# facebookresearch/multipathnet

Measured on NVIDIA H100. Metric: proposals/sec, higher is better.
Workload: dtype fp32 (wgmma split emulation, fp32 accumulate: 3 bf16 products per MAC, 2 fp16 products in fc6/fc7)

## Files before the change

multipathnet_b200/csrc/gemm_tc.cu:

```cuda
#include "conv_gemm.cuh"
#include "wgmma.cuh"
#include <algorithm>
#include <stdlib.h>
#include <string.h>

namespace {

constexpr int BM = 128;
constexpr int BK = 64;
constexpr int TC_THREADS = 384;
constexpr int CONS_THREADS = 256;
constexpr int A_TILE_BYTES = BM * BK * 2;
constexpr int SMEM_BUDGET = 196608;

__host__ __device__ constexpr int stage_bytes(int BN, bool W16 = false) { return 2 * A_TILE_BYTES + (W16 ? 1 : 2) * BN * BK * 2; }
__host__ __device__ constexpr int num_stages(int BN, bool W16 = false) {
  return (SMEM_BUDGET / stage_bytes(BN, W16)) > 4 ? 4 : (SMEM_BUDGET / stage_bytes(BN, W16));
}
__host__ __device__ constexpr int stg_ld(int BN) { return BN + 4; }
static_assert(BM * (256 + 4) * 4 <= 2 * stage_bytes(256), "staging tile must fit in the ring");

struct TcParams {
  int N, Ho, Wo, Cout;
  int kh, kw, stride, pad;
  int cblocks;
  int tn, th, tw;
  int tiles_img, tiles_h, tiles_w, tiles_n;
  const float *bias;
  const __nv_bfloat16 *res_hi, *res_lo; long long res_ld;
  __nv_bfloat16 *out_hi, *out_lo; long long out_ld;
  float *out_f32; long long out_f32_ld;
  __nv_bfloat16 *pool_hi, *pool_lo; long long pool_ld; int Hp, Wp;
  int relu;
  int splitk, kb_per_split;
  long long split_stride;
  unsigned long long *tl_min, *tl_max;
  float acc_scale;
  int out_fmt;
  unsigned *ovf;
};

__device__ __forceinline__ unsigned long long gtimer() {
  unsigned long long t; asm volatile("mov.u64 %0, %%globaltimer;" : "=l"(t)); return t;
}
__device__ __forceinline__ void tl_min_stamp(const unsigned long long *base_, int i) {
  if (base_) atomicMin(const_cast<unsigned long long *>(base_) + i, gtimer());
}
__device__ __forceinline__ void tl_max_stamp(const unsigned long long *base_, int i) {
  if (base_) atomicMax(const_cast<unsigned long long *>(base_) + i, gtimer());
}
__device__ __forceinline__ uint32_t smem_u32(const void *p) { return (uint32_t)__cvta_generic_to_shared(p); }
__device__ __forceinline__ void mbar_init(uint32_t bar, uint32_t count) {
  asm volatile("mbarrier.init.shared::cta.b64 [%0], %1;" ::"r"(bar), "r"(count) : "memory");
}
__device__ __forceinline__ void mbar_expect_tx(uint32_t bar, uint32_t bytes) {
  asm volatile("mbarrier.arrive.expect_tx.shared::cta.b64 _, [%0], %1;" ::"r"(bar), "r"(bytes) : "memory");
}
__device__ __forceinline__ void mbar_arrive(uint32_t bar) {
  asm volatile("mbarrier.arrive.shared::cta.b64 _, [%0];" ::"r"(bar) : "memory");
}
__device__ __forceinline__ void mbar_wait(uint32_t bar, uint32_t parity) {
  uint32_t done;
  uint32_t spins = 0;
  do {
    asm volatile(
        "{\n\t.reg .pred p;\n\t"
        "mbarrier.try_wait.parity.shared::cta.b64 p, [%1], %2;\n\t"
        "selp.u32 %0, 1, 0, p;\n\t}"
        : "=r"(done) : "r"(bar), "r"(parity) : "memory");
    if (!done && ++spins == (1u << 26)) __trap();
  } while (!done);
}
__device__ __forceinline__ void tma_load_4d(uint32_t dst, const CUtensorMap *tm, uint32_t bar, int c0, int c1,
                                            int c2, int c3) {
  asm volatile(
      "cp.async.bulk.tensor.4d.shared::cluster.global.mbarrier::complete_tx::bytes [%0], [%1, {%3, %4, %5, %6}], [%2];"
      ::"r"(dst), "l"(reinterpret_cast<uint64_t>(tm)), "r"(bar), "r"(c0), "r"(c1), "r"(c2), "r"(c3) : "memory");
}
__device__ __forceinline__ void tma_load_2d(uint32_t dst, const CUtensorMap *tm, uint32_t bar, int c0, int c1) {
  asm volatile(
      "cp.async.bulk.tensor.2d.shared::cluster.global.mbarrier::complete_tx::bytes [%0], [%1, {%3, %4}], [%2];"
      ::"r"(dst), "l"(reinterpret_cast<uint64_t>(tm)), "r"(bar), "r"(c0), "r"(c1) : "memory");
}
__device__ __forceinline__ void prefetch_tmap(const CUtensorMap *tm) {
  asm volatile("prefetch.tensormap [%0];" ::"l"(reinterpret_cast<uint64_t>(tm)) : "memory");
}
__device__ __forceinline__ void consumers_sync() { asm volatile("bar.sync 1, 256;" ::: "memory"); }

__device__ __forceinline__ uint64_t make_smem_desc(uint32_t saddr) {
  uint64_t d = 0;
  d |= (uint64_t)((saddr & 0x3FFFFu) >> 4);
  d |= (uint64_t)1 << 16;
  d |= (uint64_t)(1024 >> 4) << 32;
  d |= (uint64_t)1 << 62;
  return d;
}

template <int BN, bool W16>
__device__ __forceinline__ void mma_kblock(float (&acc)[BN / 2], uint64_t a_hi, uint64_t a_lo, uint64_t b_hi, uint64_t b_lo, bool first) {
#pragma unroll
  for (int k = 0; k < BK / 16; ++k) {
    const uint64_t adv = (uint64_t)((k * 16 * 2) >> 4);
    const uint32_t later = (first && k == 0) ? 0u : 1u;
    wgmma_nk16<BN, W16>(acc, a_lo + adv, b_hi + adv, later);
    if (!W16) wgmma_nk16<BN, W16>(acc, a_hi + adv, b_lo + adv, 1u);
    wgmma_nk16<BN, W16>(acc, a_hi + adv, b_hi + adv, 1u);
  }
}

template <int BN>
__device__ __forceinline__ void stage_acc(float *stg, const float (&acc)[BN / 2], int g, int t) {
  const int r0 = g * 64 + (t >> 5) * 16 + ((t & 31) >> 2), c0 = 2 * (t & 3);
#pragma unroll
  for (int j = 0; j < BN / 8; ++j) {
    *reinterpret_cast<float2 *>(stg + r0 * stg_ld(BN) + 8 * j + c0) = make_float2(acc[4 * j], acc[4 * j + 1]);
    *reinterpret_cast<float2 *>(stg + (r0 + 8) * stg_ld(BN) + 8 * j + c0) = make_float2(acc[4 * j + 2], acc[4 * j + 3]);
  }
}

template <int BN, bool W16>
__device__ __forceinline__ void epilogue_row(const TcParams &p, const float *srow, int nt, bool row_ok, long long pix,
                                             float *out_f32, int ch_first, long long ppix) {
  const bool pool = (p.pool_hi != nullptr);
  const int tile_end = min(p.Cout, nt * BN + BN);
#pragma unroll 1
  for (int ch = ch_first; ch < BN / 32; ch += 2) {
    const int col0 = nt * BN + ch * 32;
    if (col0 >= tile_end) break;
    float v[32];
#pragma unroll
    for (int j = 0; j < 8; ++j) {
      const float4 x = *reinterpret_cast<const float4 *>(srow + ch * 32 + 4 * j);
      v[4 * j] = x.x; v[4 * j + 1] = x.y; v[4 * j + 2] = x.z; v[4 * j + 3] = x.w;
    }
    if (W16) {
#pragma unroll
      for (int e = 0; e < 32; ++e) v[e] *= p.acc_scale;
    }
    if (!(row_ok || pool)) continue;
#pragma unroll
    for (int g = 0; g < 4; ++g) {
      const int c = col0 + g * 8;
      if (c >= tile_end) break;
      float f[8];
#pragma unroll
      for (int e = 0; e < 8; ++e) f[e] = v[g * 8 + e];
      const bool full8 = (c + 8 <= tile_end);
      if (p.bias) {
        if (full8) {
          const float4 b0 = __ldg(reinterpret_cast<const float4 *>(p.bias + c));
          const float4 b1 = __ldg(reinterpret_cast<const float4 *>(p.bias + c + 4));
          f[0] += b0.x; f[1] += b0.y; f[2] += b0.z; f[3] += b0.w;
          f[4] += b1.x; f[5] += b1.y; f[6] += b1.z; f[7] += b1.w;
        } else {
          for (int e = 0; e < 8 && c + e < p.Cout; ++e) f[e] += __ldg(p.bias + c + e);
        }
      }
      if (p.res_hi && full8 && row_ok) {
        const uint4 rh = *reinterpret_cast<const uint4 *>(p.res_hi + pix * p.res_ld + c);
        const uint4 rl = *reinterpret_cast<const uint4 *>(p.res_lo + pix * p.res_ld + c);
        const uint32_t hh[4] = {rh.x, rh.y, rh.z, rh.w}, ll[4] = {rl.x, rl.y, rl.z, rl.w};
#pragma unroll
        for (int t = 0; t < 4; ++t) {
          float2 x = bf16x2_to_float2(hh[t]), y = bf16x2_to_float2(ll[t]);
          f[2 * t] += x.x + y.x; f[2 * t + 1] += x.y + y.y;
        }
      }
      if (p.relu) {
#pragma unroll
        for (int e = 0; e < 8; ++e) f[e] = fmaxf(f[e], 0.f);
      }
      if (p.out_hi && full8 && row_ok) {
        uint32_t oh[4], ol[4];
#pragma unroll
        for (int t = 0; t < 4; ++t) split_x2(p.out_fmt, f[2 * t], f[2 * t + 1], oh[t], ol[t], p.ovf);
        *reinterpret_cast<uint4 *>(p.out_hi + pix * p.out_ld + c) = make_uint4(oh[0], oh[1], oh[2], oh[3]);
        *reinterpret_cast<uint4 *>(p.out_lo + pix * p.out_ld + c) = make_uint4(ol[0], ol[1], ol[2], ol[3]);
      }
      if (pool) {
#pragma unroll
        for (int e = 0; e < 8; ++e) {
          float x = row_ok ? f[e] : -INFINITY;
          x = fmaxf(x, __shfl_xor_sync(0xffffffffu, x, 1));
          x = fmaxf(x, __shfl_xor_sync(0xffffffffu, x, 8));
          f[e] = x;
        }
        if (ppix >= 0 && full8) {
          uint32_t oh[4], ol[4];
#pragma unroll
          for (int t = 0; t < 4; ++t) split_x2(p.out_fmt, f[2 * t], f[2 * t + 1], oh[t], ol[t], p.ovf);
          *reinterpret_cast<uint4 *>(p.pool_hi + ppix * p.pool_ld + c) = make_uint4(oh[0], oh[1], oh[2], oh[3]);
          *reinterpret_cast<uint4 *>(p.pool_lo + ppix * p.pool_ld + c) = make_uint4(ol[0], ol[1], ol[2], ol[3]);
        }
      }
      if (out_f32 && row_ok) {
        float *o = out_f32 + pix * p.out_f32_ld + c;
        if (full8 && ((reinterpret_cast<uintptr_t>(o) & 15) == 0)) {
          reinterpret_cast<float4 *>(o)[0] = make_float4(f[0], f[1], f[2], f[3]);
          reinterpret_cast<float4 *>(o)[1] = make_float4(f[4], f[5], f[6], f[7]);
        } else {
          for (int e = 0; e < 8 && c + e < p.Cout; ++e) o[e] = f[e];
        }
      }
    }
  }
}

template <int BN, bool W16 = false>
__global__ void __launch_bounds__(TC_THREADS, 1)
conv_gemm_tc_kernel(const __grid_constant__ CUtensorMap tmA_hi, const __grid_constant__ CUtensorMap tmA_lo,
                    const __grid_constant__ CUtensorMap tmB_hi, const __grid_constant__ CUtensorMap tmB_lo,
                    const TcParams p) {
  constexpr int S = num_stages(BN, W16);
  constexpr int STAGE = stage_bytes(BN, W16);
  constexpr int B_TILE_BYTES = BN * BK * 2;
  static_assert(BM * stg_ld(BN) * 4 <= S * STAGE, "staging tile must fit in the ring");
  extern __shared__ uint8_t smem_raw[];
  uint8_t *smem = reinterpret_cast<uint8_t *>((reinterpret_cast<uintptr_t>(smem_raw) + 1023) & ~(uintptr_t)1023);
  uint64_t *bars = reinterpret_cast<uint64_t *>(smem + (size_t)S * STAGE);
  const uint32_t smem_base = smem_u32(smem);
  const uint32_t bar_base = smem_u32(bars);
  auto full_bar = [&](int s) { return bar_base + 8u * s; };
  auto empty_bar = [&](int s) { return bar_base + 8u * (S + s); };

  const int tid = threadIdx.x, lane = tid & 31;
  const int unit = (int)blockIdx.x;
  const int tile = unit / p.splitk, split = unit - tile * p.splitk;
  const int nt = tile % p.tiles_n, mt = tile / p.tiles_n;
  const int twi = mt % p.tiles_w, thi = (mt / p.tiles_w) % p.tiles_h, tni = mt / (p.tiles_w * p.tiles_h);
  const int num_kb = p.kh * p.kw * p.cblocks;
  const int kb0 = split * p.kb_per_split, kb1 = min(num_kb, kb0 + p.kb_per_split);

  if (tid == 0) {
    tl_min_stamp(p.tl_min, 0);
    prefetch_tmap(&tmA_hi); prefetch_tmap(&tmA_lo); prefetch_tmap(&tmB_hi); prefetch_tmap(&tmB_lo);
    for (int s = 0; s < S; ++s) { mbar_init(full_bar(s), 1); mbar_init(empty_bar(s), CONS_THREADS / 32); }
    asm volatile("fence.mbarrier_init.release.cluster;" ::: "memory");
  }
  __syncthreads();
  asm volatile("griddepcontrol.wait;" ::: "memory");
  asm volatile("griddepcontrol.launch_dependents;" ::: "memory");
  if (tid == 0) tl_min_stamp(p.tl_min, 1);

  if (tid < 128) {
    if (tid == 0) {
      const int w_in0 = twi * p.tw * p.stride - p.pad, h_in0 = thi * p.th * p.stride - p.pad, n0 = tni * p.tn;
      const int b_row0 = nt * BN;
      for (int kb = kb0, it = 0; kb < kb1; ++kb, ++it) {
        const int s = it % S; const uint32_t ph = (uint32_t)(it / S) & 1u;
        mbar_wait(empty_bar(s), ph ^ 1u);
        const int tap = kb / p.cblocks, cb = kb - tap * p.cblocks;
        const int khi = tap / p.kw, kwi = tap - khi * p.kw;
        const uint32_t sa = smem_base + (uint32_t)s * STAGE;
        mbar_expect_tx(full_bar(s), (uint32_t)STAGE);
        tma_load_4d(sa, &tmA_hi, full_bar(s), cb * BK, w_in0 + kwi, h_in0 + khi, n0);
        tma_load_4d(sa + A_TILE_BYTES, &tmA_lo, full_bar(s), cb * BK, w_in0 + kwi, h_in0 + khi, n0);
        tma_load_2d(sa + 2 * A_TILE_BYTES, &tmB_hi, full_bar(s), kb * BK, b_row0);
        if (!W16) tma_load_2d(sa + 2 * A_TILE_BYTES + B_TILE_BYTES, &tmB_lo, full_bar(s), kb * BK, b_row0);
      }
    }
    return;
  }

  const int e = tid - 128;
  const int g = e >> 7, t = e & 127;
  float acc[BN / 2];
#pragma unroll
  for (int i = 0; i < BN / 2; ++i) acc[i] = 0.f;
  for (int kb = kb0, it = 0; kb < kb1; ++kb, ++it) {
    const int s = it % S; const uint32_t ph = (uint32_t)(it / S) & 1u;
    mbar_wait(full_bar(s), ph);
    if (it == 0 && e == 0) tl_min_stamp(p.tl_min, 2);
    const uint32_t sa = smem_base + (uint32_t)s * STAGE;
    const uint64_t a_hi = make_smem_desc(sa + (uint32_t)g * (A_TILE_BYTES / 2));
    const uint64_t a_lo = make_smem_desc(sa + A_TILE_BYTES + (uint32_t)g * (A_TILE_BYTES / 2));
    const uint64_t b_hi = make_smem_desc(sa + 2 * A_TILE_BYTES);
    const uint64_t b_lo = make_smem_desc(sa + 2 * A_TILE_BYTES + B_TILE_BYTES);
    wgmma_fence_acc(acc);
    wgmma_fence();
    mma_kblock<BN, W16>(acc, a_hi, a_lo, b_hi, b_lo, it == 0);
    wgmma_commit();
    wgmma_wait<1>();
    wgmma_fence_acc(acc);
    if (it > 0 && lane == 0) mbar_arrive(empty_bar((it - 1) % S));
  }
  wgmma_wait<0>();
  wgmma_fence_acc(acc);
  if (e == 0) tl_max_stamp(p.tl_max, 0);
  consumers_sync();
  float *stg = reinterpret_cast<float *>(smem);
  stage_acc<BN>(stg, acc, g, t);
  consumers_sync();

  const int row = e & 127;
  const int wl = row & (p.tw - 1), hl = (row / p.tw) & (p.th - 1), nl = row / (p.tw * p.th);
  const int wo = twi * p.tw + wl, ho = thi * p.th + hl, n = tni * p.tn + nl;
  const bool row_ok = (wo < p.Wo) && (ho < p.Ho) && (n < p.N);
  const long long pix = ((long long)n * p.Ho + ho) * p.Wo + wo;
  const long long ppix = (p.pool_hi && row_ok && !(lane & 9)) ? ((long long)n * p.Hp + (ho >> 1)) * p.Wp + (wo >> 1) : -1;
  float *const out_f32 = p.out_f32 ? p.out_f32 + (long long)split * p.split_stride : nullptr;
  epilogue_row<BN, W16>(p, stg + row * stg_ld(BN), nt, row_ok, pix, out_f32, e >> 7, ppix);
  if (e == 0) tl_max_stamp(p.tl_max, 1);
}

constexpr int C1_THREADS = 256;
constexpr int C1_B_BYTES = 2 * 64 * 128;
constexpr int C1_SMEM = 2 * A_TILE_BYTES + C1_B_BYTES + BM * stg_ld(64) * 4 + 1024;

__global__ void __launch_bounds__(C1_THREADS, 2)
conv1_tc_kernel(const float *__restrict__ x, int N, int H, int W, const float *__restrict__ w, const TcParams p) {
  extern __shared__ uint8_t smem_raw[];
  uint8_t *smem = reinterpret_cast<uint8_t *>((reinterpret_cast<uintptr_t>(smem_raw) + 1023) & ~(uintptr_t)1023);
  uint8_t *sB = smem + 2 * A_TILE_BYTES;
  float *stg = reinterpret_cast<float *>(sB + C1_B_BYTES);
  const uint32_t a_base = smem_u32(smem), b_base = smem_u32(sB);
  const int tid = threadIdx.x, lane = tid & 31;
  const int g = tid >> 7, t = tid & 127;
  const int pixels = N * H * W;
  const int total_tiles = (pixels + BM - 1) / BM;
  asm volatile("griddepcontrol.wait;" ::: "memory");
  asm volatile("griddepcontrol.launch_dependents;" ::: "memory");
  for (int i = tid; i < 64 * 4; i += C1_THREADS) {
    const int row = i >> 2, j = i & 3;
    uint32_t hh[4], ll[4];
#pragma unroll
    for (int q = 0; q < 4; ++q) {
      const int k0 = j * 8 + 2 * q;
      const float v0 = (k0 < 27) ? __ldg(w + row * 27 + k0) : 0.f, v1 = (k0 + 1 < 27) ? __ldg(w + row * 27 + k0 + 1) : 0.f;
      split_bf16x2(v0, v1, hh[q], ll[q]);
    }
    const uint32_t off = (uint32_t)row * 128u + (uint32_t)((j ^ (row & 7)) * 16);
    *reinterpret_cast<uint4 *>(sB + off) = make_uint4(hh[0], hh[1], hh[2], hh[3]);
    *reinterpret_cast<uint4 *>(sB + 64 * 128 + off) = make_uint4(ll[0], ll[1], ll[2], ll[3]);
  }
  const int HW = H * W;
  const int brow = tid & 127, bhalf = tid >> 7;
  for (int tile = blockIdx.x; tile < total_tiles; tile += gridDim.x) {
    const int pix = tile * BM + brow;
    float in[16];
#pragma unroll
    for (int k = 0; k < 16; ++k) in[k] = 0.f;
    if (pix < pixels) {
      const int n = pix / HW, rem = pix - n * HW;
      const int ho = rem / W, wo = rem - ho * W;
      const float *x0 = x + ((size_t)n * 3 * HW + (size_t)(ho - 1) * W + (wo - 1));
      const bool rok[3] = {ho >= 1, true, ho + 1 < H}, cok[3] = {wo >= 1, true, wo + 1 < W};
#pragma unroll
      for (int k = 0; k < 16; ++k) {
        const int kk = 16 * bhalf + k;
        if (kk < 27) {
          const int ci = kk / 9, r = (kk / 3) % 3, q = kk % 3;
          in[k] = (rok[r] && cok[q]) ? __ldg(x0 + ci * HW + r * W + q) : 0.f;
        }
      }
    }
    uint8_t *pa = smem + (size_t)brow * 128;
#pragma unroll
    for (int jj = 0; jj < 2; ++jj) {
      const int j = 2 * bhalf + jj;
      uint32_t hh[4], ll[4];
#pragma unroll
      for (int q = 0; q < 4; ++q) split_bf16x2(in[jj * 8 + 2 * q], in[jj * 8 + 2 * q + 1], hh[q], ll[q]);
      const int pj = (j ^ (brow & 7)) * 16;
      *reinterpret_cast<uint4 *>(pa + pj) = make_uint4(hh[0], hh[1], hh[2], hh[3]);
      *reinterpret_cast<uint4 *>(pa + A_TILE_BYTES + pj) = make_uint4(ll[0], ll[1], ll[2], ll[3]);
    }
    asm volatile("fence.proxy.async.shared::cta;" ::: "memory");
    __syncthreads();
    float acc[32];
#pragma unroll
    for (int i = 0; i < 32; ++i) acc[i] = 0.f;
    const uint64_t a_hi = make_smem_desc(a_base + (uint32_t)g * (A_TILE_BYTES / 2));
    const uint64_t a_lo = make_smem_desc(a_base + A_TILE_BYTES + (uint32_t)g * (A_TILE_BYTES / 2));
    const uint64_t b_hi = make_smem_desc(b_base), b_lo = make_smem_desc(b_base + 64 * 128);
    wgmma_fence_acc(acc);
    wgmma_fence();
#pragma unroll
    for (int k = 0; k < 2; ++k) {
      const uint64_t adv = (uint64_t)((k * 16 * 2) >> 4);
      wgmma_nk16<64, false>(acc, a_lo + adv, b_hi + adv, k ? 1u : 0u);
      wgmma_nk16<64, false>(acc, a_hi + adv, b_lo + adv, 1u);
      wgmma_nk16<64, false>(acc, a_hi + adv, b_hi + adv, 1u);
    }
    wgmma_commit();
    wgmma_wait<0>();
    wgmma_fence_acc(acc);
    stage_acc<64>(stg, acc, g, t);
    __syncthreads();
    const int row = tid & 127;
    const int opix = tile * BM + row;
    epilogue_row<64, false>(p, stg + row * stg_ld(64), 0, opix < pixels, (long long)opix, nullptr, tid >> 7, -1);
    __syncthreads();
  }
  (void)lane;
}

struct ReduceParams {
  const float *ws; long long split_stride; int splitk; long long pixels; int Cout;
  const float *bias; const __nv_bfloat16 *res_hi, *res_lo; long long res_ld; int relu;
  __nv_bfloat16 *out_hi, *out_lo; long long out_ld; float *out_f32; long long out_f32_ld;
  OutScatter scatter;
};
__global__ void __launch_bounds__(256) splitk_reduce_kernel(const ReduceParams r) {
  MPN_PDL_SYNC();
  const long long idx = (long long)blockIdx.x * blockDim.x + threadIdx.x;
  if (idx >= r.pixels * r.Cout) return;
  const long long pix = idx / r.Cout; const int c = (int)(idx - pix * r.Cout);
  float acc = 0.f;
  for (int s = 0; s < r.splitk; ++s) acc += r.ws[(long long)s * r.split_stride + idx];
  if (r.bias) acc += __ldg(r.bias + c);
  if (r.res_hi) acc += join_bf16(r.res_hi[pix * r.res_ld + c], r.res_lo[pix * r.res_ld + c]);
  if (r.relu) acc = fmaxf(acc, 0.f);
  if (r.out_hi) { __nv_bfloat16 h, l; split_bf16(acc, h, l); r.out_hi[pix * r.out_ld + c] = h; r.out_lo[pix * r.out_ld + c] = l; }
  if (r.scatter.n > 0) {
#pragma unroll 1
    for (int g = 0; g < r.scatter.n; ++g)
      if (c >= r.scatter.seg[g].c0 && c < r.scatter.seg[g].c1) { r.scatter.seg[g].ptr[pix * r.scatter.seg[g].ld + (c - r.scatter.seg[g].c0)] = acc; break; }
  } else if (r.out_f32) r.out_f32[pix * r.out_f32_ld + c] = acc;
}

typedef CUresult (*PFN_encodeTiled)(CUtensorMap *, CUtensorMapDataType, cuuint32_t, void *, const cuuint64_t *,
                                    const cuuint64_t *, const cuuint32_t *, const cuuint32_t *, CUtensorMapInterleave,
                                    CUtensorMapSwizzle, CUtensorMapL2promotion, CUtensorMapFloatOOBfill);
PFN_encodeTiled get_encode_fn() {
  static PFN_encodeTiled fn = nullptr;
  if (!fn) {
    void *p = nullptr; cudaDriverEntryPointQueryResult q;
    if (cudaGetDriverEntryPoint("cuTensorMapEncodeTiled", &p, cudaEnableDefault, &q) == cudaSuccess &&
        q == cudaDriverEntryPointSuccess)
      fn = reinterpret_cast<PFN_encodeTiled>(p);
  }
  return fn;
}

int encode_map(mpn_ctx *ctx, CUtensorMap *tm, const void *base, int rank, const cuuint64_t *dims,
               const cuuint64_t *strides_bytes , const cuuint32_t *box, const cuuint32_t *estr) {
  PFN_encodeTiled fn = get_encode_fn();
  if (!fn) return mpn_fail(ctx, MPN_ERR_CUDA, "cuTensorMapEncodeTiled entry point unavailable");
  CUresult r = fn(tm, CU_TENSOR_MAP_DATA_TYPE_BFLOAT16, (cuuint32_t)rank, const_cast<void *>(base), dims,
                  strides_bytes, box, estr, CU_TENSOR_MAP_INTERLEAVE_NONE, CU_TENSOR_MAP_SWIZZLE_128B,
                  CU_TENSOR_MAP_L2_PROMOTION_L2_256B, CU_TENSOR_MAP_FLOAT_OOB_FILL_NONE);
  if (r != CUDA_SUCCESS) {
    char b[256];
    snprintf(b, sizeof b, "cuTensorMapEncodeTiled failed (%d): rank %d dims %llu %llu box %u %u", (int)r, rank,
             (unsigned long long)dims[0], (unsigned long long)dims[1], box[0], box[1]);
    return mpn_fail(ctx, MPN_ERR_CUDA, b);
  }
  return MPN_OK;
}

inline bool tc_use_pdl() {
  static const int on = [] { const char *e = getenv("MPN_TC_PDL"); return (e && e[0] == '0') ? 0 : 1; }();
  return on != 0;
}

template <int BN, bool W16 = false>
int launch_bn(mpn_ctx *ctx, const ConvPlan &pl, const TcParams &tp) {
  const int smem = num_stages(BN, W16) * stage_bytes(BN, W16) + 1024  + 256 ;
  constexpr int slot = W16 ? 3 : (BN == 256 ? 2 : (BN == 128 ? 1 : 0));
  if (!ctx->tc_attr_set[slot]) {
    MPN_CUDA(ctx, cudaFuncSetAttribute(conv_gemm_tc_kernel<BN, W16>, cudaFuncAttributeMaxDynamicSharedMemorySize, smem));
    ctx->tc_attr_set[slot] = 1;
  }
  const long long units = (long long)pl.tiles_img * pl.tiles_h * pl.tiles_w * pl.tiles_n * pl.splitk;
  MPN_CHECK_ARG(ctx, units > 0 && units < (1ll << 31), "conv_tc: grid size out of range");
  cudaLaunchConfig_t cfg = {};
  cfg.gridDim = dim3((unsigned)units); cfg.blockDim = dim3(TC_THREADS); cfg.dynamicSmemBytes = (size_t)smem; cfg.stream = ctx->stream;
  cudaLaunchAttribute attr[1];
  int na = 0;
  if (tc_use_pdl()) {
    attr[na].id = cudaLaunchAttributeProgrammaticStreamSerialization;
    attr[na].val.programmaticStreamSerializationAllowed = 1;
    ++na;
  }
  cfg.attrs = attr; cfg.numAttrs = na;
  MPN_CUDA(ctx, cudaLaunchKernelEx(&cfg, conv_gemm_tc_kernel<BN, W16>, pl.tmA_hi, pl.tmA_lo, pl.tmB_hi, pl.tmB_lo, tp));
  MPN_LAUNCHED(ctx);
  return MPN_OK;
}

}

int conv1_tc_launch(mpn_ctx *ctx, const float *x_nchw, int N, int H, int W, const float *w_dev, const float *bias_dev, int relu,
                    DTensor &y) {
  MpnProfScope prof_scope__(ctx, MPN_CAT_CONV_DIRECT);
  MPN_CHECK_ARG(ctx, y.hi && y.lo && y.C == 64 && y.ld % 8 == 0, "conv1_tc: output must be 64-channel split planes");
  TcParams tp;
  memset(&tp, 0, sizeof(tp));
  tp.N = N; tp.Ho = H; tp.Wo = W; tp.Cout = 64; tp.bias = bias_dev; tp.relu = relu;
  tp.out_hi = y.hi; tp.out_lo = y.lo; tp.out_ld = y.ld; tp.acc_scale = 1.f;
  MPN_CHECK_ARG(ctx, y.ld == 64 && (long long)N * H * W < (1ll << 31) - 256, "conv1_tc: dense 64-channel output and < 2^31 pixels");
  if (!ctx->tc_attr_set[4]) {
    MPN_CUDA(ctx, cudaFuncSetAttribute(conv1_tc_kernel, cudaFuncAttributeMaxDynamicSharedMemorySize, C1_SMEM));
    ctx->tc_attr_set[4] = 1;
  }
  const long long tiles = ((long long)N * H * W + BM - 1) / BM;
  cudaLaunchConfig_t cfg = {};
  cfg.gridDim = dim3((unsigned)std::min<long long>(tiles, 2ll * ctx->sm_count)); cfg.blockDim = dim3(C1_THREADS);
  cfg.dynamicSmemBytes = (size_t)C1_SMEM; cfg.stream = ctx->stream;
  cudaLaunchAttribute attr[1];
  int na = 0;
  if (tc_use_pdl()) { attr[na].id = cudaLaunchAttributeProgrammaticStreamSerialization; attr[na].val.programmaticStreamSerializationAllowed = 1; ++na; }
  cfg.attrs = attr; cfg.numAttrs = na;
  MPN_CUDA(ctx, cudaLaunchKernelEx(&cfg, conv1_tc_kernel, x_nchw, N, H, W, w_dev, tp));
  MPN_LAUNCHED(ctx);
  return MPN_OK;
}

double conv_flops(const ConvProblem &p) {
  const double Ho = (double)p.y.H, Wo = (double)p.y.W;
  return 2.0 * (double)p.x.C * p.Cout * p.kh * p.kw * Ho * Wo * (double)p.y.N;
}

static int conv_tc_plan_impl(mpn_ctx *ctx, int sm_count, const ConvProblem &p, ConvPlan &pl, bool choose_only) {
  pl.valid = 0;
  MPN_CHECK_ARG(ctx, choose_only || (p.x.hi && p.x.lo && ((p.w_hi && p.w_lo) || p.w16)), "conv_tc: operands must be split-bf16 (or an fp16 weight plane)");
  pl.w16 = p.w16 ? 1 : 0;
  MPN_CHECK_ARG(ctx, choose_only || (p.x.fmt == 1) == (pl.w16 == 1), "conv_tc: fp16 activation planes go with the fp16 weight plane (and only with it)");
  MPN_CHECK_ARG(ctx, p.x.C % BK == 0, "conv_tc: Cin must be a multiple of 64");
  MPN_CHECK_ARG(ctx, p.x.ld % 8 == 0, "conv_tc: input pixel stride must be a multiple of 8 elements");
  MPN_CHECK_ARG(ctx, p.stride >= 1 && p.stride <= 2, "conv_tc: stride must be 1 or 2");
  const int Ho = (int)p.y.H, Wo = (int)p.y.W, N = (int)p.y.N;
  pl.flat = (p.kh == 1 && p.kw == 1 && p.stride == 1 && p.pad == 0) ? 1 : 0;
  pl.mode = 0; pl.splitk = 1;
  cuuint64_t dims[4], strides[3]; cuuint32_t box[4], estr[4];
  int gtn = 1, gth = 1, gtw = BM;
  if (!pl.flat) {
    double best = -1.0;
    for (int tw = 1; tw <= 128; tw <<= 1)
      for (int th = 1; th * tw <= 128; th <<= 1) {
        const int tn = 128 / (tw * th);
        if (tw * p.stride > 256 || th * p.stride > 256) continue;
        const long long tiles = (long long)((Wo + tw - 1) / tw) * ((Ho + th - 1) / th) * ((N + tn - 1) / tn);
        const double util = (double)N * Ho * Wo / (double)(tiles * 128) + 1e-6 * tw;
        if (util > best) { best = util; gtn = tn; gth = th; gtw = tw; }
      }
  }
  const long long P = (long long)p.x.N * p.x.H * p.x.W;
  {
    const bool r3_ok = (p.kh == 3 && p.kw == 3 && p.stride == 1 && p.pad == 1);
    const char *env3 = getenv("MPN_TC_R3");
    const char *env3m = getenv("MPN_TC_R3_MINPIX");
    const long long r3_minpix = env3m ? atoll(env3m) : 0;
    pl.mode = (r3_ok && !(env3 && env3[0] == '0') && P >= r3_minpix) ? 1 : 0;
  }
  const long long tiles_m = pl.flat ? (P + BM - 1) / BM
                                    : (pl.mode ? (long long)((Wo + 7) / 8) * ((Ho + 15) / 16) * N
                                               : (long long)((Wo + gtw - 1) / gtw) * ((Ho + gth - 1) / gth) * ((N + gtn - 1) / gtn));
  {
    const int taps = p.kh * p.kw;
    const double kblocks = (double)taps * (double)(p.x.C / BK);
    double best = 1e300; int best_bn = 64;
    for (int bi = 0; bi < 3; ++bi) {
      const int bn = bi == 0 ? 256 : (bi == 1 ? 128 : 64);
      if (pl.w16 && bn != 256) continue;
      if (!p.m_invariant && bn > 64 && bn > ((p.Cout + 63) / 64) * 64) continue;
      if (p.m_invariant && bn != (p.Cout > 128 ? 256 : (p.Cout > 64 ? 128 : 64))) continue;
      const long long units = tiles_m * ((p.Cout + bn - 1) / bn);
      const long long rounds = (units + sm_count - 1) / sm_count;
      const double mma = (pl.w16 ? 2.0 : 3.0) * 128.0 * bn * 64.0 / 1024.0;
      const double ingest = (pl.w16 ? 2.0 * 128 + bn : 2.0 * (128 + bn)) * 128.0 / 48.0;
      const double cost = (double)rounds * (kblocks * std::max(mma, ingest) + 1500.0 + 8.0 * bn);
      if (cost < best * 0.999) { best = cost; best_bn = bn; }
    }
    pl.BN = best_bn;
    pl.tiles_n = (p.Cout + pl.BN - 1) / pl.BN;
  }
  if (pl.flat) {
    pl.tn = 1; pl.th = 1; pl.tw = BM;
    pl.tiles_img = 1; pl.tiles_h = 1; pl.tiles_w = (int)((P + BM - 1) / BM);
    dims[0] = (cuuint64_t)p.x.C; dims[1] = (cuuint64_t)P; dims[2] = 1; dims[3] = 1;
    strides[0] = (cuuint64_t)p.x.ld * 2; strides[1] = (cuuint64_t)P * p.x.ld * 2; strides[2] = strides[1];
    box[0] = BK; box[1] = BM; box[2] = 1; box[3] = 1;
    estr[0] = estr[1] = estr[2] = estr[3] = 1;
  } else {
    if (pl.mode == 1) { pl.tn = 1; pl.th = 16; pl.tw = 8; }
    else { pl.tn = gtn; pl.th = gth; pl.tw = gtw; }
    pl.tiles_w = (Wo + pl.tw - 1) / pl.tw; pl.tiles_h = (Ho + pl.th - 1) / pl.th; pl.tiles_img = (N + pl.tn - 1) / pl.tn;
    dims[0] = (cuuint64_t)p.x.C; dims[1] = (cuuint64_t)p.x.W; dims[2] = (cuuint64_t)p.x.H; dims[3] = (cuuint64_t)p.x.N;
    strides[0] = (cuuint64_t)p.x.ld * 2; strides[1] = (cuuint64_t)p.x.W * p.x.ld * 2;
    strides[2] = (cuuint64_t)p.x.H * p.x.W * p.x.ld * 2;
    box[0] = BK; box[1] = (cuuint32_t)(pl.tw * p.stride); box[2] = (cuuint32_t)(pl.th * p.stride); box[3] = (cuuint32_t)pl.tn;
    estr[0] = 1; estr[1] = (cuuint32_t)p.stride; estr[2] = (cuuint32_t)p.stride; estr[3] = 1;
  }
  {
    const long long units = tiles_m * pl.tiles_n;
    const long long num_kb = (long long)p.kh * p.kw * (p.x.C / BK);
    long long sk = std::min<long long>(num_kb / 8, 8);
    if (p.m_invariant) { if (!(pl.flat && p.Cout <= 128) || sk < 2) sk = 1; }
    else if (pl.mode == 1 || sk < 2 || units * sk > sm_count) sk = 1;
    const char *env2 = getenv("MPN_TC_SPLITK");
    if (env2 && env2[0] == '0') sk = 1;
    pl.splitk = (int)std::max<long long>(sk, 1);
    pl.kb_per_split = (int)((num_kb + pl.splitk - 1) / pl.splitk);
    pl.splitk = (int)((num_kb + pl.kb_per_split - 1) / pl.kb_per_split);
  }
  if (choose_only) return MPN_OK;
  MPN_TRY(encode_map(ctx, &pl.tmA_hi, p.x.hi, 4, dims, strides, box, estr));
  MPN_TRY(encode_map(ctx, &pl.tmA_lo, p.x.lo, 4, dims, strides, box, estr));
  const long long Ktot = (long long)p.kh * p.kw * p.x.C;
  cuuint64_t bd[2] = {(cuuint64_t)Ktot, (cuuint64_t)p.Cout}, bs[1] = {(cuuint64_t)Ktot * 2};
  cuuint32_t bb[2] = {BK, (cuuint32_t)pl.BN}, be[2] = {1, 1};
  if (pl.w16) {
    MPN_CHECK_ARG(ctx, pl.mode == 0 && pl.flat && pl.splitk == 1 && pl.BN == 256, "conv_tc: the fp16-weight path is for wide flat GEMMs without split-K");
    MPN_TRY(encode_map(ctx, &pl.tmB_hi, p.w16, 2, bd, bs, bb, be));
    pl.tmB_lo = pl.tmB_hi;
  } else {
    MPN_TRY(encode_map(ctx, &pl.tmB_hi, p.w_hi, 2, bd, bs, bb, be));
    MPN_TRY(encode_map(ctx, &pl.tmB_lo, p.w_lo, 2, bd, bs, bb, be));
  }
  pl.valid = 1;
  return MPN_OK;
}

int conv_tc_plan(mpn_ctx *ctx, const ConvProblem &p, ConvPlan &pl) { return conv_tc_plan_impl(ctx, ctx->sm_count, p, pl, false); }

int conv_tc_launch(mpn_ctx *ctx, const ConvProblem &p, const ConvPlan &pl) {
  MpnProfScope prof_scope__(ctx, MPN_CAT_CONV_TC);
  MPN_CHECK_ARG(ctx, pl.valid, "conv_tc_launch: invalid plan");
  TcParams tp;
  memset(&tp, 0, sizeof(tp));
  if (pl.flat) { tp.N = 1; tp.Ho = 1; tp.Wo = (int)(p.y.N * p.y.H * p.y.W); }
  else { tp.N = (int)p.y.N; tp.Ho = (int)p.y.H; tp.Wo = (int)p.y.W; }
  tp.Cout = p.Cout; tp.kh = p.kh; tp.kw = p.kw; tp.stride = p.stride; tp.pad = p.pad;
  tp.cblocks = (int)(p.x.C / BK);
  tp.tn = pl.tn; tp.th = pl.th; tp.tw = pl.tw;
  tp.tiles_img = pl.tiles_img; tp.tiles_h = pl.tiles_h; tp.tiles_w = pl.tiles_w; tp.tiles_n = pl.tiles_n;
  tp.bias = p.bias;
  tp.res_hi = p.res.hi; tp.res_lo = p.res.lo; tp.res_ld = p.res.ld;
  tp.out_hi = p.y.hi; tp.out_lo = p.y.lo; tp.out_ld = p.y.ld;
  tp.out_f32 = p.y.f32; tp.out_f32_ld = p.y_f32_ld;
  tp.relu = p.relu;
  tp.splitk = pl.splitk; tp.kb_per_split = pl.kb_per_split; tp.split_stride = 0;
  tp.acc_scale = pl.w16 ? p.w16_inv_scale : 1.f;
  tp.out_fmt = p.y.fmt; tp.ovf = nullptr;
  if (p.y.fmt) MPN_TRY(mpn_ovf_flag(ctx, &tp.ovf));
  MPN_CHECK_ARG(ctx, !p.pool.hi || p.pool.fmt == p.y.fmt, "conv_tc: pooled output must share the output's plane format");
  MPN_CHECK_ARG(ctx, !(p.y.fmt && pl.splitk > 1), "conv_tc: fp16 output planes are not written by the split-K reduce");
  MPN_CHECK_ARG(ctx, !p.res.hi || p.res.fmt == 0, "conv_tc: residual inputs are bf16 split planes");
  if (ctx->tl_on && ctx->tl_n < ctx->tl_cap) { tp.tl_min = ctx->tl_min + 4 * ctx->tl_n; tp.tl_max = ctx->tl_max + 4 * ctx->tl_n; ++ctx->tl_n; }
  if (p.pool.hi) {
    MPN_CHECK_ARG(ctx, pl.mode == 1 && pl.splitk == 1 && !p.res.hi && p.Cout % 8 == 0 && p.pool.ld % 8 == 0,
                  "conv_tc: fused pooling needs the 3x3 kernel, no residual, Cout multiple of 8");
    MPN_CHECK_ARG(ctx, p.pool.H == (p.y.H + 1) / 2 && p.pool.W == (p.y.W + 1) / 2 && p.pool.N == p.y.N, "conv_tc: pooled geometry mismatch");
    tp.pool_hi = p.pool.hi; tp.pool_lo = p.pool.lo; tp.pool_ld = p.pool.ld; tp.Hp = (int)p.pool.H; tp.Wp = (int)p.pool.W;
    if (p.pool_only) { tp.out_hi = tp.out_lo = nullptr; tp.out_f32 = nullptr; }
  }
  if (p.y.hi) MPN_CHECK_ARG(ctx, p.Cout % 8 == 0 && p.y.ld % 8 == 0, "conv_tc: split output needs Cout, ld multiples of 8");
  MPN_CHECK_ARG(ctx, p.scatter.n == 0 || pl.splitk > 1, "conv_tc: scattered outputs need a split-K plan");
  if (pl.splitk > 1) {
    const long long pixels = (long long)p.y.N * p.y.H * p.y.W;
    float *ws = nullptr;
    MPN_TRY(mpn_scratch3(ctx, sizeof(float) * (size_t)pl.splitk * pixels * p.Cout, (void **)&ws));
    tp.bias = nullptr; tp.res_hi = tp.res_lo = nullptr; tp.relu = 0; tp.out_hi = tp.out_lo = nullptr;
    tp.out_f32 = ws; tp.out_f32_ld = p.Cout; tp.split_stride = pixels * p.Cout;
    const int rc = pl.BN == 256 ? launch_bn<256>(ctx, pl, tp) : (pl.BN == 128 ? launch_bn<128>(ctx, pl, tp) : launch_bn<64>(ctx, pl, tp));
    MPN_TRY(rc);
    ReduceParams r;
    r.ws = ws; r.split_stride = tp.split_stride; r.splitk = pl.splitk; r.pixels = pixels; r.Cout = p.Cout;
    r.bias = p.bias; r.res_hi = p.res.hi; r.res_lo = p.res.lo; r.res_ld = p.res.ld; r.relu = p.relu;
    r.out_hi = p.y.hi; r.out_lo = p.y.lo; r.out_ld = p.y.ld; r.out_f32 = p.y.f32; r.out_f32_ld = p.y_f32_ld;
    r.scatter = p.scatter;
    const long long total = pixels * p.Cout;
    MPN_CUDA(ctx, mpn_launch_pdl(ctx, splitk_reduce_kernel, dim3((unsigned)((total + 255) / 256)), dim3(256), 0, r));
    MPN_LAUNCHED(ctx);
    return MPN_OK;
  }
  if (pl.w16) return launch_bn<256, true>(ctx, pl, tp);
  switch (pl.BN) {
    case 256: return launch_bn<256>(ctx, pl, tp);
    case 128: return launch_bn<128>(ctx, pl, tp);
    default: return launch_bn<64>(ctx, pl, tp);
  }
}

extern "C" int mpn_debug_plan(int64_t N, int64_t Cin, int64_t H, int64_t W, int64_t Cout, int32_t k, int32_t stride, int32_t pad,
                              int32_t per_roi, int32_t sm_count, int32_t *out) {
  if (!out || N <= 0 || Cin <= 0 || Cin % 64 || H <= 0 || W <= 0 || Cout <= 0 || k <= 0 || stride < 1 || stride > 2 || pad < 0 || sm_count < 2)
    return MPN_ERR_ARG;
  ConvProblem p;
  p.x.N = N; p.x.H = H; p.x.W = W; p.x.C = Cin; p.x.ld = Cin;
  p.Cout = (int)Cout; p.kh = p.kw = k; p.stride = stride; p.pad = pad; p.m_invariant = per_roi ? 1 : 0;
  p.y.N = N; p.y.H = (H + 2 * pad - k) / stride + 1; p.y.W = (W + 2 * pad - k) / stride + 1; p.y.C = Cout; p.y.ld = Cout;
  if (p.y.H <= 0 || p.y.W <= 0) return MPN_ERR_ARG;
  ConvPlan pl;
  const int rc = conv_tc_plan_impl(nullptr, sm_count, p, pl, true);
  if (rc != MPN_OK) return rc;
  out[0] = pl.mode; out[1] = 1; out[2] = pl.BN; out[3] = pl.splitk; out[4] = 0; out[5] = pl.tn; out[6] = pl.th; out[7] = pl.tw;
  return MPN_OK;
}
```

Baseline: 277,800.

## Stage conv1 epilogue output in shared memory and write it with bulk async stores

The conv1 tensor-core kernel's epilogue now applies bias and ReLU and does the bf16 hi/lo split cooperatively, eight threads per row reading float4 pairs. It writes the result back into the A tile region of shared memory and issues cp.async.bulk stores of whole contiguous tiles to global memory. A wait on the previous bulk group before the A tile is overwritten lets each tile's output store overlap the next tile's input gather. This replaces the per-row epilogue_row path, aiming to coalesce output writes and cut store instructions. It adds a 16-byte alignment requirement, ties the kernel to a dense 64-channel layout, and removes the profiling scope from the launcher.

New measurement: 282,500, median of 6. Within noise of the previous version (+1.7%).

```diff
diff --git a/multipathnet_b200/csrc/gemm_tc.cu b/multipathnet_b200/csrc/gemm_tc.cu
--- a/multipathnet_b200/csrc/gemm_tc.cu
+++ b/multipathnet_b200/csrc/gemm_tc.cu
@@ -307,6 +307,10 @@
 constexpr int C1_B_BYTES = 2 * 64 * 128;
 constexpr int C1_SMEM = 2 * A_TILE_BYTES + C1_B_BYTES + BM * stg_ld(64) * 4 + 1024;
 
+__device__ __forceinline__ void bulk_store(void *gdst, uint32_t ssrc, uint32_t bytes) {
+  asm volatile("cp.async.bulk.global.shared::cta.bulk_group [%0], [%1], %2;" ::"l"(gdst), "r"(ssrc), "r"(bytes) : "memory");
+}
+
 __global__ void __launch_bounds__(C1_THREADS, 2)
 conv1_tc_kernel(const float *__restrict__ x, int N, int H, int W, const float *__restrict__ w, const TcParams p) {
   extern __shared__ uint8_t smem_raw[];
@@ -314,7 +318,7 @@
   uint8_t *sB = smem + 2 * A_TILE_BYTES;
   float *stg = reinterpret_cast<float *>(sB + C1_B_BYTES);
   const uint32_t a_base = smem_u32(smem), b_base = smem_u32(sB);
-  const int tid = threadIdx.x, lane = tid & 31;
+  const int tid = threadIdx.x;
   const int g = tid >> 7, t = tid & 127;
   const int pixels = N * H * W;
   const int total_tiles = (pixels + BM - 1) / BM;
@@ -333,6 +337,7 @@
     *reinterpret_cast<uint4 *>(sB + off) = make_uint4(hh[0], hh[1], hh[2], hh[3]);
     *reinterpret_cast<uint4 *>(sB + 64 * 128 + off) = make_uint4(ll[0], ll[1], ll[2], ll[3]);
   }
+  const int eg = tid & 7;
   const int HW = H * W;
   const int brow = tid & 127, bhalf = tid >> 7;
   for (int tile = blockIdx.x; tile < total_tiles; tile += gridDim.x) {
@@ -344,16 +349,19 @@
       const int n = pix / HW, rem = pix - n * HW;
       const int ho = rem / W, wo = rem - ho * W;
       const float *x0 = x + ((size_t)n * 3 * HW + (size_t)(ho - 1) * W + (wo - 1));
-      const bool rok[3] = {ho >= 1, true, ho + 1 < H}, cok[3] = {wo >= 1, true, wo + 1 < W};
+      const bool top = ho >= 1, bottom = ho + 1 < H, left = wo >= 1, right = wo + 1 < W;
 #pragma unroll
       for (int k = 0; k < 16; ++k) {
         const int kk = 16 * bhalf + k;
         if (kk < 27) {
           const int ci = kk / 9, r = (kk / 3) % 3, q = kk % 3;
-          in[k] = (rok[r] && cok[q]) ? __ldg(x0 + ci * HW + r * W + q) : 0.f;
+          const bool ok = (r == 0 ? top : (r == 2 ? bottom : true)) && (q == 0 ? left : (q == 2 ? right : true));
+          in[k] = ok ? __ldg(x0 + ci * HW + r * W + q) : 0.f;
         }
       }
     }
+    if (tid == 0) asm volatile("cp.async.bulk.wait_group.read 0;" ::: "memory");
+    __syncthreads();
     uint8_t *pa = smem + (size_t)brow * 128;
 #pragma unroll
     for (int jj = 0; jj < 2; ++jj) {
@@ -387,12 +395,38 @@
     wgmma_fence_acc(acc);
     stage_acc<64>(stg, acc, g, t);
     __syncthreads();
-    const int row = tid & 127;
-    const int opix = tile * BM + row;
-    epilogue_row<64, false>(p, stg + row * stg_ld(64), 0, opix < pixels, (long long)opix, nullptr, tid >> 7, -1);
+#pragma unroll
+    for (int i = 0; i < 4; ++i) {
+      const int row = (tid >> 3) + 32 * i;
+      const float4 v0 = *reinterpret_cast<const float4 *>(stg + row * stg_ld(64) + 8 * eg);
+      const float4 v1 = *reinterpret_cast<const float4 *>(stg + row * stg_ld(64) + 8 * eg + 4);
+      float f[8] = {v0.x, v0.y, v0.z, v0.w, v1.x, v1.y, v1.z, v1.w};
+      if (p.bias) {
+        const float4 b0 = __ldg(reinterpret_cast<const float4 *>(p.bias + 8 * eg));
+        const float4 b1 = __ldg(reinterpret_cast<const float4 *>(p.bias + 8 * eg + 4));
+        f[0] += b0.x; f[1] += b0.y; f[2] += b0.z; f[3] += b0.w;
+        f[4] += b1.x; f[5] += b1.y; f[6] += b1.z; f[7] += b1.w;
+      }
+      if (p.relu) {
+#pragma unroll
+        for (int e = 0; e < 8; ++e) f[e] = fmaxf(f[e], 0.f);
+      }
+      uint32_t oh[4], ol[4];
+#pragma unroll
+      for (int q = 0; q < 4; ++q) split_bf16x2(f[2 * q], f[2 * q + 1], oh[q], ol[q]);
+      *reinterpret_cast<uint4 *>(smem + row * 128 + 16 * eg) = make_uint4(oh[0], oh[1], oh[2], oh[3]);
+      *reinterpret_cast<uint4 *>(smem + A_TILE_BYTES + row * 128 + 16 * eg) = make_uint4(ol[0], ol[1], ol[2], ol[3]);
+    }
+    asm volatile("fence.proxy.async.shared::cta;" ::: "memory");
     __syncthreads();
-  }
-  (void)lane;
+    if (tid == 0) {
+      const uint32_t bytes = (uint32_t)min(BM, pixels - tile * BM) * 128u;
+      bulk_store(p.out_hi + (size_t)tile * BM * 64, a_base, bytes);
+      bulk_store(p.out_lo + (size_t)tile * BM * 64, a_base + A_TILE_BYTES, bytes);
+      asm volatile("cp.async.bulk.commit_group;" ::: "memory");
+    }
+  }
+  if (tid == 0) asm volatile("cp.async.bulk.wait_group 0;" ::: "memory");
 }
 
 struct ReduceParams {
@@ -483,13 +517,14 @@
 
 int conv1_tc_launch(mpn_ctx *ctx, const float *x_nchw, int N, int H, int W, const float *w_dev, const float *bias_dev, int relu,
                     DTensor &y) {
-  MpnProfScope prof_scope__(ctx, MPN_CAT_CONV_DIRECT);
   MPN_CHECK_ARG(ctx, y.hi && y.lo && y.C == 64 && y.ld % 8 == 0, "conv1_tc: output must be 64-channel split planes");
   TcParams tp;
   memset(&tp, 0, sizeof(tp));
   tp.N = N; tp.Ho = H; tp.Wo = W; tp.Cout = 64; tp.bias = bias_dev; tp.relu = relu;
   tp.out_hi = y.hi; tp.out_lo = y.lo; tp.out_ld = y.ld; tp.acc_scale = 1.f;
   MPN_CHECK_ARG(ctx, y.ld == 64 && (long long)N * H * W < (1ll << 31) - 256, "conv1_tc: dense 64-channel output and < 2^31 pixels");
+  MPN_CHECK_ARG(ctx, ((reinterpret_cast<uintptr_t>(y.hi) | reinterpret_cast<uintptr_t>(y.lo)) & 15) == 0,
+                "conv1_tc: output planes must be 16-byte aligned (bulk-copy stores)");
   if (!ctx->tc_attr_set[4]) {
     MPN_CUDA(ctx, cudaFuncSetAttribute(conv1_tc_kernel, cudaFuncAttributeMaxDynamicSharedMemorySize, C1_SMEM));
     ctx->tc_attr_set[4] = 1;
```
